# ssteinberg/wave_tracer

Measured on AMD Instinct MI355X. Metric: Msamples/sec (whole node), cornell-box 1440^2 wave-mode, higher is better.
Workload: dtype f32

## Files before the change

wave_tracer_amd/api.py:

```python
import ctypes as C
import json
import math
import os

_HERE = os.path.dirname(os.path.abspath(__file__))

os.environ.setdefault("HSA_KERNARG_POOL_SIZE", str(16 << 20))


def lib_path():
    return os.environ.get("WTGPU_LIB") or os.path.join(_HERE, "libwtgpu.so")


class WtgpuError(RuntimeError):
    pass


class SceneParams(C.Structure):
    _fields_ = [("res", C.c_uint32), ("max_depth", C.c_int32), ("fsd", C.c_int32), ("mis", C.c_int32), ("rr", C.c_int32),
                ("force_ray_tracing", C.c_int32), ("mesh_detail", C.c_int32), ("lut_n_theta", C.c_uint32), ("lut_m", C.c_uint32),
                ("polarimetric", C.c_int32)]


class TestHooks(C.Structure):
# ... 113 lines not shown
    lib.wtgpu_scene_compare_part.argtypes = [vp, vp, C.c_char_p, C.c_char_p, C.c_size_t]
    lib.wtgpu_trace_ab_stats.argtypes = [vp, C.POINTER(C.c_double), C.POINTER(C.c_double), C.POINTER(u64), C.POINTER(u64), C.POINTER(u64)]
    lib.wtgpu_render_progressive.argtypes = [vp, vp, vp, vp, vp, u64, u64, u64, u32, PROGRESS_CB, vp, C.POINTER(u64)]
    lib.wtgpu_cancel.argtypes = [vp]
    lib.wtgpu_pause.argtypes = [vp]
    lib.wtgpu_resume.argtypes = [vp]
    lib.wtgpu_capture_intermediate.argtypes = [vp, CAPTURE_CB, vp]
    lib.wtgpu_comm_unique_id.argtypes = [vp]
    lib.wtgpu_comm_create.argtypes = [i32, i32, i32, vp, C.POINTER(vp)]
    lib.wtgpu_film_reduce.argtypes = [vp, vp, vp, vp, vp, u64, u64, i32]
    lib.wtgpu_comm_destroy.argtypes = [vp]
    lib.wtgpu_comm_destroy.restype = None
    lib.wtgpu_scene_get_info.argtypes = [vp, C.POINTER(SceneInfo)]
    lib.wtgpu_scene_host_desc.argtypes = [vp]
    lib.wtgpu_scene_host_desc.restype = vp
    lib.wtgpu_scene_upload.argtypes = [vp, i32, u64]
    lib.wtgpu_render.argtypes = [vp, vp, vp, vp, vp, u64, u64, u64]
    lib.wtgpu_render_async.argtypes = [vp, vp, vp, vp, vp, u64, u64, u64]
    lib.wtgpu_join.argtypes = [vp, vp]
    lib.wtgpu_trace_rays.argtypes = [vp, vp, vp, u32, vp, vp, vp, vp]
    lib.wtgpu_traverse_cones.argtypes = [vp, vp, vp, u32, u32, vp, vp, vp, vp]
    lib.wtgpu_query_regions.argtypes = [vp, vp, vp, u32, u32, vp, vp, vp, vp, vp, vp, vp]
    lib.wtgpu_test_fsd_apertures.argtypes = [vp, vp, vp, vp, vp, vp, u32, u32, u32, u32, vp, vp]
    lib.wtgpu_test_utd_sums.argtypes = [vp, vp, vp, vp, vp, u32, u32, u32, vp, vp, vp]
    lib.wtgpu_test_profile_counters.argtypes = [vp, vp, u32]
    lib.wtgpu_test_bsdf_queries.argtypes = [vp, vp, vp, u32, i32, vp]
    lib.wtgpu_test_source_queries.argtypes = [vp, vp, vp, u32, vp]
    lib.wtgpu_scene_shape_id.argtypes = [vp, u32, C.POINTER(C.c_char_p)]
    lib.wtgpu_scene_sensor_mask_spec.argtypes = [vp, C.POINTER(SensorMaskSpec)]
    lib.wtgpu_sensor_mask.argtypes = [vp, vp, vp, u32, u64, vp]
    lib.wtgpu_sensor_mask_host.argtypes = [vp, vp, u32, u64, u32, vp]
    lib.wtgpu_scene_tonemap_spec.argtypes = [vp, C.POINTER(TonemapSpec)]
    lib.wtgpu_develop_device.argtypes = [vp, vp, vp, vp, vp, u64, vp]
    lib.wtgpu_tonemap_device.argtypes = [vp, vp, vp, vp, vp, u64, C.POINTER(Tonemap), u32, vp, u32, vp]
    lib.wtgpu_tonemap_host.argtypes = [vp, vp, vp, vp, u64, C.POINTER(Tonemap), u32, vp, u32, u32, vp]
    lib.wtgpu_film_stats_edges.argtypes = [C.POINTER(FilmStatsSpec), vp]
    lib.wtgpu_film_stats_device.argtypes = [vp, vp, vp, vp, vp, u64, C.POINTER(FilmStatsSpec), vp, vp, vp]
    lib.wtgpu_film_stats_host.argtypes = [vp, vp, vp, vp, u64, C.POINTER(FilmStatsSpec), vp, u32, vp, vp]
    lib.wtgpu_film_compare_device.argtypes = [vp, vp, vp, vp, vp, u64, vp, vp, vp, u64, C.POINTER(FilmCompareSpec), vp, vp, vp]
    lib.wtgpu_film_compare_host.argtypes = [vp, vp, vp, vp, u64, vp, vp, vp, u64, C.POINTER(FilmCompareSpec), vp, u32, vp, vp]
    lib.wtgpu_calibrate_copy.argtypes = [u64, i32]
    lib.wtgpu_get_counters.argtypes = [vp, C.POINTER(Counters)]
    lib.wtgpu_reset_counters.argtypes = [vp]
    lib.wtgpu_last_render_timings.argtypes = [vp, C.POINTER(C.c_float * 12)]
    lib.wtgpu_develop.argtypes = [vp, vp, vp, vp, u64, vp]
    lib.wtgpu_scene_destroy.argtypes = [vp]
# ... 173 lines not shown
        _check(load_library().wtgpu_traverse_cones(self._h, None, d_cones.data_ptr(), n, cap, dist.data_ptr(), flags.data_ptr(), ntris.data_ptr(),
                                                   tris.data_ptr()))
        torch.cuda.synchronize(dev)
        return (dist.cpu().numpy(), flags.cpu().numpy().view(np.uint32), ntris.cpu().numpy().view(np.uint32),
                tris.cpu().numpy().view(np.uint32))

    def query_regions(self, cones, edge_cap=96):
        import numpy as np
        import torch
        dev = torch.device("cuda", self.device)
        n = len(cones)
        d_cones = torch.from_numpy(np.ascontiguousarray(cones, dtype=np.float32)).to(dev)
        dist = torch.zeros(n, dtype=torch.float32, device=dev)
        flux = torch.zeros(n, dtype=torch.float32, device=dev)
        flags, primary, ntris, nedges = (torch.zeros(n, dtype=torch.int32, device=dev) for _ in range(4))
        edges = torch.full((n, edge_cap), -1, dtype=torch.int32, device=dev)
        _check(load_library().wtgpu_query_regions(self._h, None, d_cones.data_ptr(), n, edge_cap, dist.data_ptr(), flags.data_ptr(), primary.data_ptr(),
                                                  ntris.data_ptr(), nedges.data_ptr(), edges.data_ptr(), flux.data_ptr()))
        torch.cuda.synchronize(dev)
        u = lambda t: t.cpu().numpy().view(np.uint32)
        return {"dist": dist.cpu().numpy(), "flags": u(flags), "primary": u(primary), "ntris": u(ntris), "nedges": u(nedges), "edges": u(edges),
                "flux": flux.cpu().numpy()}

    def fsd_apertures(self, cones, sk, ids, n_ids, pool_cap=4096, mode=0):
        import numpy as np
        import torch
        dev = torch.device("cuda", self.device)
        ids = np.ascontiguousarray(ids, dtype=np.uint32)
        n, id_cap = ids.shape
        n_ids = np.ascontiguousarray(n_ids, dtype=np.uint32)
        assert len(cones) == n and len(sk) == n and len(n_ids) == n and (n_ids <= id_cap).all()
        n_edges = self.info.n_edges
        assert all((ids[i, :n_ids[i]] < n_edges).all() for i in range(n)), "edge id out of range"
        t = lambda a, dt: torch.from_numpy(np.ascontiguousarray(a, dtype=dt)).to(dev)
        d_cones, d_sk = t(cones, np.float32), t(sk, np.float32)
        d_ids, d_nids = t(ids.view(np.int32), np.int32), t(n_ids.view(np.int32), np.int32)
        hdr = torch.zeros((n, 8), dtype=torch.int32, device=dev)
        segs = torch.zeros((n, pool_cap, 7), dtype=torch.float32, device=dev)
        _check(load_library().wtgpu_test_fsd_apertures(self._h, None, d_cones.data_ptr(), d_sk.data_ptr(), d_ids.data_ptr(), d_nids.data_ptr(), n, id_cap,
                                                       pool_cap, mode, hdr.data_ptr(), segs.data_ptr()))
        torch.cuda.synchronize(dev)
        return hdr.cpu().numpy().view(np.uint32), segs.cpu().numpy()

    def utd_sums(self, queries, ids, n_ids, utd_cap=48):
        import numpy as np
        import torch
# ... 356 lines not shown
```

wave_tracer_amd/csrc/kernels_trace.hip:

```cpp
#include "wtgpu_kernels.h"

namespace wtk {

}
#include "kernels_trace_refill.h"
namespace wtk {

__global__ void __launch_bounds__(kBlock, WTGPU_LB_TRACE) k_trace_refill(launch_args_t a, int in, int first_round, uint32_t round) { trace_refill_body(a, in, first_round, round); }

#ifndef WTGPU_SM_EXACT_MIN
#define WTGPU_SM_EXACT_MIN 24
#endif
#ifndef WTGPU_SM_SPLIT_NODE
#define WTGPU_SM_SPLIT_NODE 0
#endif
#ifndef WTGPU_SM_BOTH
#define WTGPU_SM_BOTH 0
#endif
enum : int { PH_IDLE = 0, PH_NODE = 1, PH_TRI = 2, PH_EXACT = 3, PH_SERVE = 4, PH_POLICY = 5, PH_RAYDONE = 6 };
#ifdef WTGPU_SM_PROF
#define SP_DECL() unsigned long long sp_t[8] = {0, 0, 0, 0, 0, 0, 0, 0}, sp_l[8] = {0, 0, 0, 0, 0, 0, 0, 0}, sp_n[8] = {0, 0, 0, 0, 0, 0, 0, 0}; long long sp_c = 0
#define SP_BEGIN() sp_c = clock64()
#define SP_END(i, mask) do { const long long d_ = clock64() - sp_c; sp_t[i] += (unsigned long long)d_; sp_l[i] += (unsigned long long)d_ * (unsigned long long)__popcll(mask); sp_n[i] += 1; } while (0)
#else
// ... 769 lines not shown
        const range_t izr{tr.dist, tr.dist + tr.region_depth};
        prim = tr.tuid;
        const vec2 ax = cone_axes(env, tr.dist);
        ge = coop_gather(sc, env, izr, env, cone_frame(env), izr, vec2{1.f, 1.f}, false, gsh, false, true, nullptr, 1, &eg);
        __syncthreads();
        if (sc.n_edges <= kCoopEdgeBits) {
            ge.n_edges = coop_edge_count(sc, eg);
            coop_edge_write(sc, eg, edges + (size_t)i * edge_cap, edge_cap);
        } else
            for (uint32_t j = threadIdx.x; j < ge.n_edges && j < edge_cap; j += 64) edges[(size_t)i * edge_cap + j] = eg.edge_ids[j];
        __syncthreads();
        gf = coop_gather(sc, env, izr, env, cone_frame(env), izr, vec2{ax.x / kBeamEnvelope, ax.y / kBeamEnvelope}, tr.front_face != 0, gsh, true, false);
    }
    if (threadIdx.x == 0) {
        dist[i] = tr.dist;
        flags[i] = (tr.empty ? 1u : 0u) | (tr.ballistic ? 2u : 0u) | (tr.front_face ? 4u : 0u);
        primary[i] = prim;
        ntris[i] = gf.n_tris;
        nedges[i] = ge.n_edges + ge.edge_overflow;
        flux[i] = (float)gf.flux;
    }
}

}
```

wave_tracer_amd/csrc/wt/coop.h:

```cpp
#pragma once
#if defined(__HIPCC__)
#include "bvh.h"
#include "gauss.h"

namespace wt {

constexpr int kCoopStack = 512;
#ifndef WTGPU_COOP_LEAF_TRIS
#define WTGPU_COOP_LEAF_TRIS 256
#endif
constexpr uint32_t kCoopLeafTris = WTGPU_COOP_LEAF_TRIS;
constexpr uint32_t kCoopGatherLeafTris = 64;
constexpr uint32_t kCoopTriBuf = 64 + 8 * kCoopLeafTris;

#ifndef WTGPU_COOP_FLUSH_AT
#define WTGPU_COOP_FLUSH_AT 12
#endif
constexpr uint32_t kCoopFlushAt = WTGPU_COOP_FLUSH_AT;
constexpr uint32_t kCoopSurvCap = 128;

#ifndef WT_COOP_SPHERES
#define WT_COOP_SPHERES 1
#endif
#ifndef WT_COOP_SPHERE_PREFETCH
#define WT_COOP_SPHERE_PREFETCH 1
#endif
constexpr uint32_t kCoopSpherePrefetch = WT_COOP_SPHERE_PREFETCH;
WT_D const float4* coop_tri_spheres(const scene_t& sc) { return reinterpret_cast<const float4*>(sc.tri_geo + sc.n_tris); }
struct coop_shared_t {
    unsigned long long* dropped;
    stack_entry_t stack[kCoopStack];
    uint32_t tri_buf[kCoopTriBuf];
    uint32_t surv[kCoopSurvCap];
    float hit_dist[64];
};
struct coop_gather_shared_t {
    unsigned long long* dropped;
    stack_entry_t stack[kCoopStack];
    uint32_t tri_buf[64 + 8 * 64];
    uint32_t surv[kCoopSurvCap];
};
struct coop_edges_t {
    uint32_t edge_ids[96];
    uint32_t edge_bits[1024];
};
constexpr uint32_t kCoopEdgeBits = 32768;

template <class SH>
WT_D void coop_set_dropped_counter(SH& sh, unsigned long long* slot) {
    if (threadIdx.x == 0) sh.dropped = slot;
    __syncthreads();
}
WT_D float wave_min(float v) {
#pragma unroll
    for (int off = 32; off > 0; off >>= 1) v = fminf(v, __shfl_xor(v, off, 64));
    return v;
}
WT_D int uniform(int x) { return __builtin_amdgcn_readfirstlane(x); }
WT_D uint32_t uniform(uint32_t x) { return (uint32_t)__builtin_amdgcn_readfirstlane((int)x); }
WT_D bool uniform(bool x) { return __builtin_amdgcn_readfirstlane((int)x) != 0; }
WT_D float uniform(float x) { return __int_as_float(__builtin_amdgcn_readfirstlane(__float_as_int(x))); }
WT_D vec3 uniform(vec3 v) { return vec3{uniform(v.x), uniform(v.y), uniform(v.z)}; }
WT_D range_t uniform(const range_t& r) { return range_t{uniform(r.min), uniform(r.max)}; }
WT_D cone_t uniform(const cone_t& c) {
    cone_t u;
    u.o = uniform(c.o);
    u.d = uniform(c.d);
    u.x = uniform(c.x);
    u.x0 = uniform(c.x0);
    u.tan_alpha = uniform(c.tan_alpha);
    u.e = uniform(c.e);
    u.one_over_e = uniform(c.one_over_e);
    u.z_apex = uniform(c.z_apex);
    return u;
}

WT_D void coop_tri_vertices(const scene_t& sc, uint32_t tuid, vec3& a, vec3& b, vec3& c) {
    const float4* q = reinterpret_cast<const float4*>(sc.tri_geo + tuid);
    const float4 q0 = q[0], q1 = q[1];
    const float q2 = reinterpret_cast<const float*>(q)[8];
    a = vec3{q0.x, q0.y, q0.z};
    b = vec3{q0.w, q1.x, q1.y};
    c = vec3{q1.z, q1.w, q2};
}

WT_D bool cone_child_test(const bvh8_node_t& n, int i, vec3 ro, vec3 rd, vec3 rinvd, bool sx, bool sy, bool sz, float ta, float ix,
                                       const range_t& range, float& tmin_out) {
    float ominx = n.minx[i] - ro.x, ominy = n.miny[i] - ro.y, ominz = n.minz[i] - ro.z;
    float omaxx = n.maxx[i] - ro.x, omaxy = n.maxy[i] - ro.y, omaxz = n.maxz[i] - ro.z;
    const bool outside = cone_box_outside(ominx, ominy, ominz, omaxx, omaxy, omaxz, rd, ta, ix, range);
    const float bx = sx ? ominx : omaxx, by = sy ? ominy : omaxy, bz = sz ? ominz : omaxz;
    const float dot_d_b = rd.x * bx + rd.y * by + rd.z * bz;
    const float maxz = clampf(dot_d_b, 0.f, range.max);
    const float enlr = fmaf(maxz, ta, ix);
    ominx -= enlr;
    ominy -= enlr;
    ominz -= enlr;
    omaxx += enlr;
    omaxy += enlr;
    omaxz += enlr;
    const float dminx = (sx ? omaxx : ominx) * rinvd.x, dmaxx = (sx ? ominx : omaxx) * rinvd.x;
    const float dminy = (sy ? omaxy : ominy) * rinvd.y, dmaxy = (sy ? ominy : omaxy) * rinvd.y;
    const float dminz = (sz ? omaxz : ominz) * rinvd.z, dmaxz = (sz ? ominz : omaxz) * rinvd.z;
    float tmin = 0.f, tmax = dmaxx;
    tmin = fmaxf_(tmin, dminx);
    tmax = fminf_(tmax, dmaxy);
    tmin = fmaxf_(tmin, dminy);
    tmax = fminf_(tmax, dmaxz);
    tmin = fmaxf_(tmin, dminz);
    tmin_out = tmin;
    return !outside && tmin <= tmax && tmax >= range.min && tmin <= range.max && !(tmin >= range.max);
}

template <bool any_hit>
WT_D bool coop_cone_query(const scene_t& sc, const cone_t& cone_, const range_t& searchrange_, float z_scale, coop_shared_t& sh,
                                       const uint_list_t& tris, cone_hit_t& rec, unsigned long long* prof = nullptr, float min_progress_ = -WT_INF) {
    const cone_t cone = uniform(cone_);
    const range_t searchrange = uniform(searchrange_);
    const float min_progress = uniform(min_progress_);
    const int lane = threadIdx.x & 63;
    const int grp = lane >> 3, sub = lane & 7;
    rec.dist = WT_INF;
    rec.front_face = 0;
    rec.ntris = 0;
    rec.overflow = 0;
    rec.aborted = 0;
    rec.too_short = 0;
    rec.short_tuid = kInvalid;
    if (sc.n_nodes == 0) return false;
    const vec3 ro = cone.o, rd = cone.d;
    const vec3 rinvd = uniform(vec3{1.f / rd.x, 1.f / rd.y, 1.f / rd.z});
    const bool sx = __builtin_signbit(rinvd.x), sy = __builtin_signbit(rinvd.y), sz = __builtin_signbit(rinvd.z);
    const float ta = cone.tan_alpha, ix = cone.x0;
    range_t range = any_hit ? searchrange : uniform(cone_search_range(cone, searchrange, rec.dist, z_scale));
    float slab_max = range.max;
    int s = 1;
    uint32_t leaf_total = 0, nsurv = 0;
    if (lane == 0) sh.stack[0] = stack_entry_t{0.f, 1};
    __syncthreads();
    auto compact = [&](float zmax) __attribute__((always_inline)) {
        if (rec.ntris == 0) return;
        __syncthreads();
        const bool mine = (uint32_t)lane < rec.ntris;
        const uint32_t val = mine ? tris[lane] : 0u;
        const float dv = mine ? sh.hit_dist[lane] : 0.f;
        const bool keep = mine && !(dv > zmax);
        const unsigned long long km = __ballot(keep);
        __syncthreads();
        if (keep) {
            const uint32_t np_ = (uint32_t)__popcll(km & ((1ull << lane) - 1ull));
            tris[np_] = val;
            sh.hit_dist[np_] = dv;
        }
        rec.ntris = (uint32_t)__popcll(km);
        __syncthreads();
    };
    auto flush = [&]() __attribute__((always_inline)) -> bool {
        __syncthreads();
        bool any = false;
        for (uint32_t b2 = 0; b2 < nsurv && !any; b2 += 64) {
// ... 105 lines not shown
            CP(1);
            const unsigned long long hm = __ballot(h);
            if (hm) {
                const uint32_t gbits = (uint32_t)(hm >> (grp * 8)) & 0xffu;
                int rank = 0;
#pragma unroll
                for (int j = 0; j < 8; ++j) {
                    const float tj = __shfl(tmin, (lane & ~7) + j, 64);
                    if (((gbits >> j) & 1u) && (tj > tmin || (tj == tmin && j < sub))) ++rank;
                }
                const int above = grp < 7 ? __popcll(hm >> ((grp + 1) * 8)) : 0;
                const int pos = s + above + rank;
                if (h && pos < kCoopStack) sh.stack[pos] = stack_entry_t{tmin, cp};
                else if (h) atomicAdd(sh.dropped, 1ull);
                const int total = s + __popcll(hm);
                s = total < kCoopStack ? total : kCoopStack;
            }
            CP(2);
            const unsigned long long lm = __ballot(leafish && sub == 0 && cnt > 0);
            unsigned long long m = lm;
            while (m) {
                const int src = __ffsll((long long)m) - 1;
                m &= m - 1;
                uint32_t c = uniform((uint32_t)__shfl((int)cnt, src, 64));
                const uint32_t t = uniform((uint32_t)__shfl((int)t0, src, 64));
                if (c > kCoopLeafTris) c = kCoopLeafTris;
                for (uint32_t q = (uint32_t)lane; q < c; q += 64u) sh.tri_buf[leaf_total + q] = t + q;
                leaf_total += c;
            }
            __syncthreads();
            CP(3);
        }
        if (prof) prof[5] += (unsigned long long)(clock64() - ta0);
        const long long tb0 = prof ? clock64() : 0;
        bool found_any = false;
#ifdef WTGPU_COOP_PROF
        if (prof) { prof[10] += 1; prof[11] += leaf_total; prof[8] += (leaf_total + 63u) / 64u; }
#endif
#if WT_COOP_SPHERES
        {
            const float4* spheres = coop_tri_spheres(sc);
            uint32_t n2 = 0;
            for (uint32_t base0 = 0; base0 < leaf_total; base0 += 64u * kCoopSpherePrefetch) {
                float4 bs[kCoopSpherePrefetch];
                uint32_t tu[kCoopSpherePrefetch];
#pragma unroll
                for (uint32_t j = 0; j < kCoopSpherePrefetch; ++j) {
                    const uint32_t k = base0 + 64u * j + lane;
                    tu[j] = 0;
                    bs[j] = float4{0.f, 0.f, 0.f, 0.f};
                    if (k < leaf_total) {
                        tu[j] = sh.tri_buf[k];
                        bs[j] = spheres[tu[j]];
                    }
                }
#pragma unroll
                for (uint32_t j = 0; j < kCoopSpherePrefetch; ++j) asm volatile("" : "+v"(bs[j].x), "+v"(bs[j].y), "+v"(bs[j].z), "+v"(bs[j].w));
                __syncthreads();
#pragma unroll
                for (uint32_t j = 0; j < kCoopSpherePrefetch; ++j) {
                    const uint32_t k = base0 + 64u * j + lane;
// ... 8 lines not shown
            CP(7);
        }
#endif
        for (uint32_t base = 0; base < leaf_total && !found_any; base += 64) {
            const uint32_t k = base + lane;
            bool pass = false;
            uint32_t tuid = 0;
            if (k < leaf_total) {
                tuid = sh.tri_buf[k];
                vec3 va, vb, vc;
                coop_tri_vertices(sc, tuid, va, vb, vc);
                pass = cone_tri_maybe(cone, va, vb, vc, range);
            }
            const unsigned long long pm = __ballot(pass);
            if (pm) {
                const uint32_t pos = nsurv + (uint32_t)__popcll(pm & ((1ull << lane) - 1ull));
                if (pass && pos < kCoopSurvCap) sh.surv[pos] = tuid;
                nsurv += (uint32_t)__popcll(pm);
            }
            CP(7);
            if (nsurv >= 64u) found_any = flush();
            CP(6);
        }
        leaf_total = 0;
        CP(7);
        if (!found_any && nsurv > 0 && (s == 0 || nsurv >= kCoopFlushAt)) found_any = flush();
        CP(6);
        __syncthreads();
        if (prof) prof[6] += (unsigned long long)(clock64() - tb0);
        if (found_any && (any_hit || rec.too_short)) return true;
        if (s == 0) break;
    }
    return rec.ntris > 0;
}

WT_D void coop_cone(const scene_t& sc, const cone_t& cone, const range_t& searchrange, float z_scale, coop_shared_t& sh,
                                 const uint_list_t& tris, cone_hit_t& rec, unsigned long long* prof = nullptr, float min_progress = -WT_INF) {
    coop_cone_query<false>(sc, cone, searchrange, z_scale, sh, tris, rec, prof, min_progress);
}
WT_D bool coop_cone_any(const scene_t& sc, const cone_t& cone, const range_t& range, coop_shared_t& sh, unsigned long long* prof = nullptr,
                                     uint32_t* hit_tuid = nullptr) {
    cone_hit_t rec;
    const uint_list_t none{nullptr, 0, 0};
    const bool hit = coop_cone_query<true>(sc, cone, range, 0.f, sh, none, rec, prof);
    if (hit_tuid) *hit_tuid = rec.short_tuid;
    return hit;
}

struct gather_out_t {
    double flux;
    uint32_t n_edges, edge_overflow;
    uint32_t n_tris;
};
template <class SH>
WT_D gather_out_t coop_gather(const scene_t& sc, const cone_t& tcone, const range_t& slab, const cone_t& envelope, const frame_t& beam_frame,
                                           const range_t& izr, vec2 sigma, bool want_front, SH& sh, bool do_flux, bool do_edges,
                                           unsigned long long* stats = nullptr, int32_t root = 1, coop_edges_t* eg = nullptr) {
    uint32_t* edges = eg ? eg->edge_ids : nullptr;
    const uint32_t edge_cap = 96;
    const int lane = threadIdx.x & 63;
    const int grp = lane >> 3, sub = lane & 7;
    gather_out_t out{0.0, 0u, 0u, 0u};
    const bool edges_only = do_edges && !do_flux;
// ... 229 lines not shown
        float tmin = 0.f;
        if (grp < np) {
            const bvh8_node_t& node = sc.nodes[e.ptr - 1];
            cp = node.child[sub];
            if (cp != 0 && cone_child_test(node, sub, ro, rd, rinvd, sx, sy, sz, ta, ix, slab, tmin)) {
                if (cp < 0 || sc.nodes[cp - 1].tris_count <= max_tris)
                    emit(cp);
                else
                    push = true;
            }
        }
        const unsigned long long hm = __ballot(push);
        if (hm) {
            const int pos = s + __popcll(hm & ((1ull << lane) - 1ull));
            if (push && pos < kCoopStack) sh.stack[pos] = stack_entry_t{tmin, cp};
            else if (push) emit(cp);
            const int total = s + __popcll(hm);
            s = total < kCoopStack ? total : kCoopStack;
        }
        __syncthreads();
    }
}

WT_D bool coop_ray_query(const scene_t& sc, vec3 ro_, vec3 rd_, const range_t& range_, coop_shared_t& sh, ray_hit_t& rec) {
    const vec3 ro = uniform(ro_), rd = uniform(rd_);
    const range_t range = uniform(range_);
    const int lane = threadIdx.x & 63;
    const int grp = lane >> 3, sub = lane & 7;
    rec.dist = WT_INF;
    rec.tuid = kInvalid;
    rec.bx = rec.by = 0.f;
    rec.front_face = 0;
    if (sc.n_nodes == 0) return false;
    const vec3 rinvd = uniform(vec3{1.f / rd.x, 1.f / rd.y, 1.f / rd.z});
    const bool sx = __builtin_signbit(rinvd.x), sy = __builtin_signbit(rinvd.y), sz = __builtin_signbit(rinvd.z);
    int s = 1;
    uint32_t leaf_total = 0;
    if (lane == 0) sh.stack[0] = stack_entry_t{0.f, 1};
    __syncthreads();
    for (;;) {
        while (s > 0 && leaf_total < 64u) {
            const int np = s < 8 ? s : 8;
            stack_entry_t e{0.f, 0};
            if (grp < np) e = sh.stack[s - 1 - grp];
            s -= np;
            __syncthreads();
            const bool live = grp < np && e.t < rec.dist;
            bool leafish = false, h = false;
            uint32_t t0 = 0, cnt = 0;
            float tmin = 0.f;
            int32_t cp = 0;
            if (live) {
                if (e.ptr < 0) {
                    const bvh8_leaf_t leaf = bvh_leaf_of(e.ptr);
                    t0 = leaf.tris_ptr;
                    cnt = leaf.count;
                    leafish = true;
                } else {
                    const bvh8_node_t& n = sc.nodes[e.ptr - 1];
                    const uint32_t ntc = n.tris_count, nts = n.tris_start;
// ... 21 lines not shown
                }
            }
            const unsigned long long hm = __ballot(h);
            if (hm) {
                const uint32_t gbits = (uint32_t)(hm >> (grp * 8)) & 0xffu;
                int rank = 0;
#pragma unroll
                for (int j = 0; j < 8; ++j) {
                    const float tj = __shfl(tmin, (lane & ~7) + j, 64);
                    if (((gbits >> j) & 1u) && (tj > tmin || (tj == tmin && j < sub))) ++rank;
                }
                const int above = grp < 7 ? __popcll(hm >> ((grp + 1) * 8)) : 0;
                const int pos = s + above + rank;
                if (h && pos < kCoopStack) sh.stack[pos] = stack_entry_t{tmin, cp};
                else if (h) atomicAdd(sh.dropped, 1ull);
                const int total = s + __popcll(hm);
                s = total < kCoopStack ? total : kCoopStack;
            }
            const unsigned long long lm = __ballot(leafish && sub == 0 && cnt > 0);
            unsigned long long m = lm;
            while (m) {
                const int src = __ffsll((long long)m) - 1;
                m &= m - 1;
                uint32_t c = uniform((uint32_t)__shfl((int)cnt, src, 64));
                const uint32_t t = uniform((uint32_t)__shfl((int)t0, src, 64));
                if (c > kCoopLeafTris) c = kCoopLeafTris;
                for (uint32_t q = (uint32_t)lane; q < c; q += 64u) sh.tri_buf[leaf_total + q] = t + q;
                leaf_total += c;
            }
            __syncthreads();
        }
        if (leaf_total == 0) {
            if (s == 0) break;
            continue;
        }
        for (uint32_t base = 0; base < leaf_total; base += 64) {
            const uint32_t k = base + lane;
            bool hit = false;
            float d = WT_INF;
            uint32_t tuid = 0;
            ray_tri_hit_t ht{WT_INF, 0.f, 0.f};
            bool ff = false;
            if (k < leaf_total) {
                tuid = sh.tri_buf[k];
                const tri_geo_t tri = sc.tri_geo[tuid];
                if (intersect_ray_tri_wide(ro, rd, tri.a, tri.b, tri.c, range, ht) && ht.dist < rec.dist) {
                    hit = true;
                    d = ht.dist;
                    ff = dot(tri.n, rd) <= 0.f;
                }
            }
            const unsigned long long mask = __ballot(hit);
            if (mask) {
                const float dm = uniform(wave_min(d));
                const unsigned long long m2 = __ballot(hit && d == dm);
                const int src = __ffsll((long long)m2) - 1;
                rec.dist = dm;
                rec.tuid = uniform((uint32_t)__shfl((int)tuid, src, 64));
                rec.bx = uniform(__shfl(ht.bx, src, 64));
                rec.by = uniform(__shfl(ht.by, src, 64));
                rec.front_face = uniform((uint32_t)__shfl((int)ff, src, 64));
            }
        }
        leaf_total = 0;
        __syncthreads();
        if (s == 0) break;
    }
    if (!finitef(rec.dist) || rec.dist > range.max) {
        rec.dist = WT_INF;
        return false;
    }
    return true;
}

WT_D trav_result_t coop_traverse(const scene_t& sc, const cone_t& envelope_, float lambda_m_, float distance_, bool force_ray_tracing,
                                              coop_shared_t& sh, const uint_list_t& tris, unsigned long long* prof = nullptr, bool resume = false,
                                              uint32_t seg0_ = 0, float dist0 = 0.f, uint32_t nray0 = 0, uint32_t ncone0 = 0, const ray_hit_t* axis = nullptr,
                                              bool primary_always = false, bool probe_resumed = true, uint32_t short_tuid_ = kInvalid,
                                              uint32_t origin_tuid_ = kInvalid, bool use_cache = true) {
    const cone_t envelope = uniform(envelope_);
    const float lambda_m = uniform(lambda_m_), distance = uniform(distance_);
    const uint32_t seg0 = uniform(seg0_), origin_tuid = uniform(origin_tuid_);
    uint32_t short_tuid = uniform(short_tuid_);
#ifdef WTGPU_COOP_PROF
#define WT_COOP_PROF(i, t0_)
#else
#define WT_COOP_PROF(i, t0_) \
    if (prof) prof[i] += (unsigned long long)(clock64() - (t0_));
#endif
    trav_result_t r;
    r.aborted = 0;
    r.origin = envelope.o;
    r.empty = 1;
    r.ballistic = 1;
    r.dist = -WT_INF;
    r.region_depth = 0.f;
    r.front_face = 0;
    r.tuid = kInvalid;
    r.bx = r.by = 0.f;
// ... 91 lines not shown
```

wave_tracer_amd/csrc/wtgpu_kernels.h:

```cpp
#pragma once
#include <hip/hip_runtime.h>

#include <cstddef>
#include <cstdint>
#include <cstring>

#include "../../include/wtgpu.h"
#include "wt/bdpt.h"
#include "wt/coop.h"
#include "wt/coop_fsd.h"
#include "wt/coop_utd.h"
#include "wt/path.h"

using namespace wt;
namespace wt {
struct tonemap_args_t;
}

namespace wtk {


#ifndef WTGPU_LB_TRACE
#define WTGPU_LB_TRACE 3
#endif
// ... 297 lines not shown
__global__ void k_path_fsd(launch_args_t a, const path_state_t* __restrict__ ps, uint32_t round);
__global__ void k_path_edges(launch_args_t a, const path_state_t* __restrict__ ps);
__global__ void k_path_interact(launch_args_t a, const path_state_t* __restrict__ ps, int in, int first_round, uint32_t round);
__global__ void k_path_interact_b(launch_args_t a, const path_state_t* __restrict__ ps, int in, uint32_t round);
__global__ void k_path_nee(launch_args_t a, const path_state_t* __restrict__ ps, uint32_t round);
__global__ void k_path_flush(launch_args_t a, int in);
__global__ void k_connect_enum(launch_args_t a, uint32_t by_class);
__global__ void k_connect_scan(launch_args_t a, uint32_t by_class);
__global__ void k_connect_strat(launch_args_t a);
__global__ void k_connect_strat_open(launch_args_t a);
__global__ void k_connect_class(launch_args_t a);
__global__ void k_connect_class_open(launch_args_t a);
__global__ void k_connect_eval(launch_args_t a, uint32_t chunk);
__global__ void k_connect_shadow(launch_args_t a, uint32_t chunk);
__global__ void k_connect_mis(launch_args_t a, uint32_t chunk);
__global__ void k_connect_splat(launch_args_t a);
__global__ void k_connect_splat_tiled(launch_args_t a);
__global__ void k_calib_copy(const uint32_t* in, uint32_t* out, size_t n);
__global__ void k_trace_rays(scene_t sc, const float* rays, uint32_t n, float* dist, uint32_t* tuid, float* bary, uint32_t* front);
__global__ void k_traverse_cones(scene_t sc, const float* cones, uint32_t n, uint32_t cap, float* dist, uint32_t* flags, uint32_t* ntris, uint32_t* out_tris,
                                 uint32_t* scratch_tris);
__global__ void k_query_regions(scene_t sc, const float* cones, uint32_t n, uint32_t edge_cap, float* dist, uint32_t* flags, uint32_t* primary, uint32_t* ntris,
                                uint32_t* nedges, uint32_t* edges, float* flux, unsigned long long* dropped);
int test_fsd_apertures(const scene_t& sc, hipStream_t stream, const float* d_cones, const float* d_sk, const uint32_t* d_ids, const uint32_t* d_n_ids,
                       uint32_t n, uint32_t id_cap, uint32_t pool_cap, uint32_t mode, uint32_t* d_hdr, float* d_segs);
int test_utd_sums(const scene_t& sc, hipStream_t stream, const float* d_queries, const uint32_t* d_ids, const uint32_t* d_n_ids, uint32_t n, uint32_t id_cap,
                  uint32_t utd_cap, uint32_t* d_recs, uint32_t* d_hdr, uint32_t* d_edges);
int test_bsdf_queries(const scene_t& sc, hipStream_t stream, const uint32_t* d_queries, uint32_t n, int form, uint32_t* d_out);
int test_source_queries(const scene_t& sc, hipStream_t stream, const uint32_t* d_queries, uint32_t n, uint32_t* d_out);
int sensor_mask_launch(const scene_t& sc, hipStream_t stream, const uint8_t* d_shape_matches, uint32_t samples, uint64_t seed, float* d_out);
void sensor_mask_host(const scene_t& sc, const uint8_t* shape_matches, uint32_t samples, uint64_t seed, uint32_t n_threads, float* out);
constexpr uint32_t kMaxTonemapTable = 1024;
int develop_launch(const sensor_t& sn, hipStream_t stream, const double* d_value, const double* d_weight, const double* d_light, uint64_t spe,
                   uint32_t per_pixel, float* d_out);
int develop_tonemap_launch(const sensor_t& sn, hipStream_t stream, const double* d_value, const double* d_weight, const double* d_light, uint64_t spe,
                           const tonemap_args_t& t, uint32_t s, const float* d_mask, uint32_t format, uint32_t lds_table, void* d_out);
void develop_tonemap_host(const sensor_t& sn, const double* value, const double* weight, const double* light, uint64_t spe, const tonemap_args_t& t, uint32_t s,
                          const float* mask, uint32_t format, uint32_t n_threads, void* out);
int film_stats_launch(const sensor_t& sn, hipStream_t stream, uint32_t n_cus, const double* d_value, const double* d_weight, const double* d_light, uint64_t spe, uint32_t s,
                      uint32_t flags, const float* d_mask, const float* d_edges, uint32_t bins, void* d_rec, unsigned long long* d_hist, double* d_sums);
void film_stats_host(const sensor_t& sn, const double* value, const double* weight, const double* light, uint64_t spe, uint32_t s, uint32_t flags, const float* mask,
                     const float* edges, uint32_t bins, uint32_t n_threads, void* out_rec, unsigned long long* out_hist);
size_t film_compare_wave_bytes(uint64_t npix, uint32_t n_cus);
int film_compare_launch(const sensor_t& sn, hipStream_t stream, uint32_t n_cus, const double* a_value, const double* a_weight, const double* a_light, uint64_t spe_a,
                        const double* b_value, const double* b_weight, const double* b_light, uint64_t spe_b, uint32_t s, uint32_t flags, double eps, const float* d_mask,
                        void* d_rec, double* d_sums, void* d_wave, float* d_diff);
// ... 7 lines not shown
```

wave_tracer_amd/csrc/wtgpu_queries.hip:

```cpp
#include "wtgpu_host.h"
#include "wt/sources_probe.h"

extern "C" {

int wtgpu_trace_rays(wtgpu_scene* s, void* stream_, const float* d_rays, uint32_t n, float* d_dist, uint32_t* d_tuid, float* d_bary, uint32_t* d_front) {
    if (!s || !s->uploaded) return fail(WTGPU_ERR_INVALID, "scene not uploaded");
    hipStream_t stream = static_cast<hipStream_t>(stream_);
    hipLaunchKernelGGL(k_trace_rays, dim3((n + kBlock - 1) / kBlock), dim3(kBlock), 0, stream, s->dev, d_rays, n, d_dist, d_tuid, d_bary, d_front);
    HIP_CHECK(hipGetLastError());
    return WTGPU_OK;
}
int wtgpu_traverse_cones(wtgpu_scene* s, void* stream_, const float* d_cones, uint32_t n, uint32_t cap, float* d_dist, uint32_t* d_flags,
                         uint32_t* d_ntris, uint32_t* d_tris) {
    if (!s || !s->uploaded) return fail(WTGPU_ERR_INVALID, "scene not uploaded");
    hipStream_t stream = static_cast<hipStream_t>(stream_);
    const size_t need = (size_t)n * kMaxConeTris * 4 * 2;
    if (need > s->query_scratch_bytes) {
        device_guard_t guard(s->device);
        void* p = nullptr;
        HIP_CHECK(hipMalloc(&p, need));
        s->dev_allocs.push_back(p);
        s->query_scratch = static_cast<uint32_t*>(p);
        s->query_scratch_bytes = need;
    }
    hipLaunchKernelGGL(k_traverse_cones, dim3((n + kBlock - 1) / kBlock), dim3(kBlock), 0, stream, s->dev, d_cones, n, cap, d_dist, d_flags, d_ntris,
                       d_tris, s->query_scratch);
    HIP_CHECK(hipGetLastError());
    return WTGPU_OK;
}

int wtgpu_query_regions(wtgpu_scene* s, void* stream_, const float* d_cones, uint32_t n, uint32_t edge_cap, float* d_dist, uint32_t* d_flags,
                        uint32_t* d_primary, uint32_t* d_ntris, uint32_t* d_nedges, uint32_t* d_edges, float* d_flux) {
    if (!s || !s->uploaded) return fail(WTGPU_ERR_INVALID, "scene not uploaded");
    if (n == 0) return WTGPU_OK;
    hipLaunchKernelGGL(k_query_regions, dim3(n), dim3(64), 0, static_cast<hipStream_t>(stream_), s->dev, d_cones, n, edge_cap, d_dist, d_flags, d_primary,
                       d_ntris, d_nedges, d_edges, d_flux, s->slices[0].counters + kDroppedSlot);
    HIP_CHECK(hipGetLastError());
    return WTGPU_OK;
}

int wtgpu_scene_shape_id(const wtgpu_scene* s, uint32_t shape, const char** id) {
    if (!s || !id) return fail(WTGPU_ERR_INVALID, "null argument");
    if (shape >= s->host.n_shapes) return fail(WTGPU_ERR_INVALID, "shape index out of range");
    *id = shape < s->file.shape_ids.size() ? s->file.shape_ids[shape].c_str() : "";
    return WTGPU_OK;
}
int wtgpu_scene_sensor_mask_spec(const wtgpu_scene* s, wtgpu_sensor_mask_spec* out) {
    if (!s || !out) return fail(WTGPU_ERR_INVALID, "null argument");
    out->present = s->file.has_mask ? 1 : 0;
    out->samples = s->file.mask_samples;
    out->regex = s->file.mask_regex.c_str();
    out->shape_flags = s->file.has_mask && !s->file.mask_flags.empty() ? s->file.mask_flags.data() : nullptr;
    out->n_shapes = s->host.n_shapes;
    return WTGPU_OK;
}
static int mask_flags_for(const wtgpu_scene* s, const uint8_t* shape_flags, uint32_t samples, const uint8_t** flags) {
    if (s->host.sensor.type != SENSOR_PERSPECTIVE)
        return fail(WTGPU_ERR_INVALID, "sensor masks need a perspective sensor (only the perspective loader reads a <sensor_mask>: src/sensor/perspective.cpp:98)");
    if (samples == 0 || samples > 65536) return fail(WTGPU_ERR_INVALID, "sensor mask: 1 .. 65536 samples per pixel expected");
// ... 126 lines not shown
```

wave_tracer_amd/csrc/wtgpu_test_hooks.h:

```cpp
#pragma once
#include "../../include/wtgpu.h"
#ifdef __cplusplus
extern "C" {
#endif
typedef struct wtgpu_test_hooks {
    uint32_t only_s, only_t;
    uint32_t crop_of;
} wtgpu_test_hooks;
int wtgpu_scene_create_named_hooks(const char* name, const wtgpu_scene_params* params, const wtgpu_test_hooks* hooks, wtgpu_scene** out);
int wtgpu_scene_compare(const wtgpu_scene* a, const wtgpu_scene* b, char* what, size_t n_what);
int wtgpu_scene_compare_part(const wtgpu_scene* a, const wtgpu_scene* b, const char* part, char* what, size_t n_what);
int wtgpu_trace_ab_stats(wtgpu_scene* s, double* ms_refill, double* ms_sm, uint64_t* differing_words, uint64_t* walks, uint64_t* rounds);
int wtgpu_test_profile_counters(wtgpu_scene* s, unsigned long long* out, uint32_t n);
int wtgpu_test_fsd_apertures(wtgpu_scene* s, void* stream, const float* d_cones, const float* d_sk, const uint32_t* d_ids, const uint32_t* d_n_ids,
                             uint32_t n, uint32_t id_cap, uint32_t pool_cap, uint32_t mode, uint32_t* d_hdr, float* d_segs);
int wtgpu_test_utd_sums(wtgpu_scene* s, void* stream, const float* d_queries, const uint32_t* d_ids, const uint32_t* d_n_ids, uint32_t n, uint32_t id_cap,
                        uint32_t utd_cap, uint32_t* d_recs, uint32_t* d_hdr, uint32_t* d_edges);
int wtgpu_test_bsdf_queries(wtgpu_scene* s, void* stream, const uint32_t* d_queries, uint32_t n, int form, uint32_t* d_out);
int wtgpu_test_source_queries(wtgpu_scene* s, void* stream, const uint32_t* d_queries, uint32_t n, uint32_t* d_out);
int wtgpu_test_connect_class_order(uint32_t* keys, uint32_t cap, uint32_t* n_keys, uint32_t* key_dim);
int wtgpu_test_connect_class_items(wtgpu_scene* s, uint32_t slice, uint32_t* table, uint32_t* items, uint32_t items_cap, uint32_t* n_items);
#ifdef __cplusplus
}
#endif
```

Before: 32.65.

## Replace explicit per-leaf triangle id buffer with wave-register leaf ranges in coop traversal

```diff
diff --git a/wave_tracer_amd/api.py b/wave_tracer_amd/api.py
--- a/wave_tracer_amd/api.py
+++ b/wave_tracer_amd/api.py
@@ -159,6 +159,8 @@
     lib.wtgpu_traverse_cones.argtypes = [vp, vp, vp, u32, u32, vp, vp, vp, vp]
     lib.wtgpu_query_regions.argtypes = [vp, vp, vp, u32, u32, vp, vp, vp, vp, vp, vp, vp]
     lib.wtgpu_test_fsd_apertures.argtypes = [vp, vp, vp, vp, vp, vp, u32, u32, u32, u32, vp, vp]
+    if hasattr(lib, "wtgpu_test_heavy_queries"):
+        lib.wtgpu_test_heavy_queries.argtypes = [vp, vp, vp, u32, i32, vp, vp]
     lib.wtgpu_test_utd_sums.argtypes = [vp, vp, vp, vp, vp, u32, u32, u32, vp, vp, vp]
     lib.wtgpu_test_profile_counters.argtypes = [vp, vp, u32]
     lib.wtgpu_test_bsdf_queries.argtypes = [vp, vp, vp, u32, i32, vp]
@@ -378,6 +380,20 @@
         return {"dist": dist.cpu().numpy(), "flags": u(flags), "primary": u(primary), "ntris": u(ntris), "nedges": u(nedges), "edges": u(edges),
                 "flux": flux.cpu().numpy()}
 
+    def heavy_queries(self, queries, parent_form=False):
+        import numpy as np
+        import torch
+        dev = torch.device("cuda", self.device)
+        q = np.ascontiguousarray(queries, dtype=np.float32)
+        assert q.ndim == 2 and q.shape[1] == 16
+        n = len(q)
+        d_q = torch.from_numpy(q).to(dev)
+        out = torch.zeros((n, 8), dtype=torch.int32, device=dev)
+        tris = torch.zeros((n, 64), dtype=torch.int32, device=dev)
+        _check(load_library().wtgpu_test_heavy_queries(self._h, None, d_q.data_ptr(), n, int(bool(parent_form)), out.data_ptr(), tris.data_ptr()))
+        torch.cuda.synchronize(dev)
+        return out.cpu().numpy().view(np.uint32), tris.cpu().numpy().view(np.uint32)
+
     def fsd_apertures(self, cones, sk, ids, n_ids, pool_cap=4096, mode=0):
         import numpy as np
         import torch
diff --git a/wave_tracer_amd/csrc/kernels_trace.hip b/wave_tracer_amd/csrc/kernels_trace.hip
--- a/wave_tracer_amd/csrc/kernels_trace.hip
+++ b/wave_tracer_amd/csrc/kernels_trace.hip
@@ -815,4 +815,51 @@
     }
 }
 
-}
+template <class SH>
+WT_D void test_heavy_query(const scene_t& sc, const float* q, uint32_t i, uint32_t* out, uint32_t* tris, SH& sh) {
+    const float* c = q + 16 * (size_t)i;
+    const vec3 d = normalize(vec3{c[3], c[4], c[5]});
+    const cone_t env = uniform(make_cone(vec3{c[0], c[1], c[2]}, d, build_orthogonal_frame(d).t, c[6], c[8], c[7]));
+    const uint_list_t list{tris + (size_t)i * kMaxConeTris, 1u, kMaxConeTris};
+    for (uint32_t j = threadIdx.x; j < kMaxConeTris; j += 64) list[j] = kInvalid;
+    __syncthreads();
+    uint32_t o[8] = {0, 0, 0, 0, 0, kInvalid, 0, 0};
+    if (c[10] == 0.f) {
+        const trav_result_t tr = coop_traverse(sc, env, uniform(c[9]), WT_INF, false, sh, list);
+        o[0] = __float_as_uint(tr.dist);
+        o[1] = (tr.empty ? 1u : 0u) | (tr.ballistic ? 2u : 0u) | (tr.front_face ? 4u : 0u);
+        o[2] = tr.ballistic ? 0u : tr.ntris;
+        o[3] = tr.overflow;
+        o[6] = tr.n_cone_queries;
+        o[7] = tr.n_ray_queries;
+    } else {
+        cone_hit_t rec;
+        coop_cone_query<false>(sc, env, range_t{uniform(c[11]), uniform(c[12])}, kMajorAxisToZScale, sh, list, rec, nullptr, uniform(c[13]));
+        o[0] = __float_as_uint(rec.dist);
+        o[1] = rec.front_face ? 4u : 0u;
+        o[2] = rec.ntris;
+        o[3] = rec.overflow;
+        o[4] = rec.too_short;
+        o[5] = rec.short_tuid;
+        o[6] = 1;
+    }
+    __syncthreads();
+    for (uint32_t j = threadIdx.x; j < kMaxConeTris; j += 64)
+        if (j >= o[2]) list[j] = kInvalid;
+    if (threadIdx.x == 0)
+        for (int j = 0; j < 8; ++j) out[8 * (size_t)i + j] = o[j];
+}
+__global__ void __launch_bounds__(64) k_test_heavy_queries(scene_t sc, const float* q, uint32_t n, uint32_t* out, uint32_t* tris, unsigned long long* dropped) {
+    __shared__ coop_shared_t sh;
+    coop_set_dropped_counter(sh, dropped);
+    if (blockIdx.x < n) test_heavy_query(sc, q, blockIdx.x, out, tris, sh);
+}
+#if WTGPU_COOP_PARENT_FORM
+__global__ void __launch_bounds__(64) k_test_heavy_queries_ids(scene_t sc, const float* q, uint32_t n, uint32_t* out, uint32_t* tris, unsigned long long* dropped) {
+    __shared__ coop_shared_ids_t sh;
+    coop_set_dropped_counter(sh, dropped);
+    if (blockIdx.x < n) test_heavy_query(sc, q, blockIdx.x, out, tris, sh);
+}
+#endif
+
+}
diff --git a/wave_tracer_amd/csrc/wt/coop.h b/wave_tracer_amd/csrc/wt/coop.h
--- a/wave_tracer_amd/csrc/wt/coop.h
+++ b/wave_tracer_amd/csrc/wt/coop.h
@@ -27,13 +27,28 @@
 #endif
 constexpr uint32_t kCoopSpherePrefetch = WT_COOP_SPHERE_PREFETCH;
 WT_D const float4* coop_tri_spheres(const scene_t& sc) { return reinterpret_cast<const float4*>(sc.tri_geo + sc.n_tris); }
+constexpr uint32_t kCoopCandCap = 128;
 struct coop_shared_t {
+    static constexpr bool kExplicitIds = false;
+    unsigned long long* dropped;
+    stack_entry_t stack[kCoopStack];
+    uint32_t cand[kCoopCandCap];
+    uint32_t surv[kCoopSurvCap];
+    float hit_dist[64];
+};
+#ifndef WTGPU_COOP_PARENT_FORM
+#define WTGPU_COOP_PARENT_FORM 1
+#endif
+#if WTGPU_COOP_PARENT_FORM
+struct coop_shared_ids_t {
+    static constexpr bool kExplicitIds = true;
     unsigned long long* dropped;
     stack_entry_t stack[kCoopStack];
     uint32_t tri_buf[kCoopTriBuf];
     uint32_t surv[kCoopSurvCap];
     float hit_dist[64];
 };
+#endif
 struct coop_gather_shared_t {
     unsigned long long* dropped;
     stack_entry_t stack[kCoopStack];
@@ -74,6 +89,43 @@
     u.z_apex = uniform(c.z_apex);
     return u;
 }
+
+struct coop_ranges_t {
+    uint32_t t0 = 0, s0 = 0, t1 = 0, s1 = 0;
+    uint32_t n = 0;
+    uint32_t cur = 0;
+    WT_D void clear() { n = cur = 0; }
+    WT_D void push(uint32_t first, uint32_t start, int lane) {
+        const bool mine = (uint32_t)lane == (n & 63u);
+        if (n < 64u) {
+            t0 = mine ? first : t0;
+            s0 = mine ? start : s0;
+        } else {
+            t1 = mine ? first : t1;
+            s1 = mine ? start : s1;
+        }
+        ++n;
+    }
+    WT_D uint32_t first(uint32_t r) const {
+        return (uint32_t)(r < 64u ? __builtin_amdgcn_readlane((int)t0, (int)r) : __builtin_amdgcn_readlane((int)t1, (int)(r - 64u) & 63));
+    }
+    WT_D uint32_t start(uint32_t r, uint32_t total) const {
+        if (r >= n) return total;
+        return (uint32_t)(r < 64u ? __builtin_amdgcn_readlane((int)s0, (int)r) : __builtin_amdgcn_readlane((int)s1, (int)(r - 64u) & 63));
+    }
+    WT_D uint32_t fetch(uint32_t base, uint32_t total, int lane) {
+        const uint32_t k = base + (uint32_t)lane, bend = base + 64u < total ? base + 64u : total;
+        uint32_t tu = 0;
+        while (cur < n) {
+            const uint32_t S = start(cur, total), E = start(cur + 1u, total), T = first(cur);
+            if (k >= S && k < E) tu = T + (k - S);
+            if (E > bend) break;
+            ++cur;
+            if (E == bend) break;
+        }
+        return tu;
+    }
+};
 
 WT_D void coop_tri_vertices(const scene_t& sc, uint32_t tuid, vec3& a, vec3& b, vec3& c) {
     const float4* q = reinterpret_cast<const float4*>(sc.tri_geo + tuid);
@@ -112,8 +164,8 @@
     return !outside && tmin <= tmax && tmax >= range.min && tmin <= range.max && !(tmin >= range.max);
 }
 
-template <bool any_hit>
-WT_D bool coop_cone_query(const scene_t& sc, const cone_t& cone_, const range_t& searchrange_, float z_scale, coop_shared_t& sh,
+template <bool any_hit, class SH>
+WT_D bool coop_cone_query(const scene_t& sc, const cone_t& cone_, const range_t& searchrange_, float z_scale, SH& sh,
                                        const uint_list_t& tris, cone_hit_t& rec, unsigned long long* prof = nullptr, float min_progress_ = -WT_INF) {
     const cone_t cone = uniform(cone_);
     const range_t searchrange = uniform(searchrange_);
@@ -136,6 +188,7 @@
     float slab_max = range.max;
     int s = 1;
     uint32_t leaf_total = 0, nsurv = 0;
+    coop_ranges_t rg;
     if (lane == 0) sh.stack[0] = stack_entry_t{0.f, 1};
     __syncthreads();
     auto compact = [&](float zmax) __attribute__((always_inline)) {
@@ -287,11 +340,18 @@
             while (m) {
                 const int src = __ffsll((long long)m) - 1;
                 m &= m - 1;
-                uint32_t c = uniform((uint32_t)__shfl((int)cnt, src, 64));
-                const uint32_t t = uniform((uint32_t)__shfl((int)t0, src, 64));
-                if (c > kCoopLeafTris) c = kCoopLeafTris;
-                for (uint32_t q = (uint32_t)lane; q < c; q += 64u) sh.tri_buf[leaf_total + q] = t + q;
-                leaf_total += c;
+                if constexpr (SH::kExplicitIds) {
+                    uint32_t c = uniform((uint32_t)__shfl((int)cnt, src, 64));
+                    const uint32_t t = uniform((uint32_t)__shfl((int)t0, src, 64));
+                    if (c > kCoopLeafTris) c = kCoopLeafTris;
+                    for (uint32_t q = (uint32_t)lane; q < c; q += 64u) sh.tri_buf[leaf_total + q] = t + q;
+                    leaf_total += c;
+                } else {
+                    uint32_t c = (uint32_t)__builtin_amdgcn_readlane((int)cnt, src);
+                    if (c > kCoopLeafTris) c = kCoopLeafTris;
+                    rg.push((uint32_t)__builtin_amdgcn_readlane((int)t0, src), leaf_total, lane);
+                    leaf_total += c;
+                }
             }
             __syncthreads();
             CP(3);
@@ -302,6 +362,57 @@
 #ifdef WTGPU_COOP_PROF
         if (prof) { prof[10] += 1; prof[11] += leaf_total; prof[8] += (leaf_total + 63u) / 64u; }
 #endif
+        if constexpr (!SH::kExplicitIds) {
+            const float4* spheres = coop_tri_spheres(sc);
+            const range_t range_a = range;
+            uint32_t ncand = 0, chead = 0;
+            auto filter_batch = [&](uint32_t nb) __attribute__((always_inline)) {
+                __syncthreads();
+                bool pass = false;
+                uint32_t tuid = 0;
+                if ((uint32_t)lane < nb) {
+                    tuid = sh.cand[(chead + (uint32_t)lane) & (kCoopCandCap - 1u)];
+                    vec3 va, vb, vc;
+                    coop_tri_vertices(sc, tuid, va, vb, vc);
+                    pass = cone_tri_maybe(cone, va, vb, vc, range);
+                }
+                __syncthreads();
+                const unsigned long long pm = __ballot(pass);
+                if (pm) {
+                    const uint32_t pos = nsurv + (uint32_t)__popcll(pm & ((1ull << lane) - 1ull));
+                    if (pass && pos < kCoopSurvCap) sh.surv[pos] = tuid;
+                    nsurv += (uint32_t)__popcll(pm);
+                }
+                CP(7);
+                if (nsurv >= 64u) found_any = flush();
+                CP(6);
+            };
+            for (uint32_t base0 = 0; !found_any; base0 += 64u) {
+                const bool more = base0 < leaf_total;
+                if (more) {
+                    const uint32_t tu = rg.fetch(base0, leaf_total, lane);
+                    bool p1 = base0 + (uint32_t)lane < leaf_total;
+#if WT_COOP_SPHERES
+                    float4 bs{0.f, 0.f, 0.f, 0.f};
+                    if (p1) bs = spheres[tu];
+                    asm volatile("" : "+v"(bs.x), "+v"(bs.y), "+v"(bs.z), "+v"(bs.w));
+                    p1 = p1 && cone_sphere_maybe(cone, vec3{bs.x, bs.y, bs.z}, bs.w, range_a);
+#endif
+                    const unsigned long long pm1 = __ballot(p1);
+                    if (p1) sh.cand[(chead + ncand + (uint32_t)__popcll(pm1 & ((1ull << lane) - 1ull))) & (kCoopCandCap - 1u)] = tu;
+                    ncand += (uint32_t)__popcll(pm1);
+                    CP(7);
+                }
+                if (ncand >= 64u || (!more && ncand > 0)) {
+                    const uint32_t nb = ncand < 64u ? ncand : 64u;
+                    filter_batch(nb);
+                    chead = (chead + nb) & (kCoopCandCap - 1u);
+                    ncand -= nb;
+                }
+                if (!more) break;
+            }
+            rg.clear();
+        } else {
 #if WT_COOP_SPHERES
         {
             const float4* spheres = coop_tri_spheres(sc);
@@ -356,6 +467,7 @@
             if (nsurv >= 64u) found_any = flush();
             CP(6);
         }
+        }
         leaf_total = 0;
         CP(7);
         if (!found_any && nsurv > 0 && (s == 0 || nsurv >= kCoopFlushAt)) found_any = flush();
@@ -368,11 +480,13 @@
     return rec.ntris > 0;
 }
 
-WT_D void coop_cone(const scene_t& sc, const cone_t& cone, const range_t& searchrange, float z_scale, coop_shared_t& sh,
+template <class SH>
+WT_D void coop_cone(const scene_t& sc, const cone_t& cone, const range_t& searchrange, float z_scale, SH& sh,
                                  const uint_list_t& tris, cone_hit_t& rec, unsigned long long* prof = nullptr, float min_progress = -WT_INF) {
     coop_cone_query<false>(sc, cone, searchrange, z_scale, sh, tris, rec, prof, min_progress);
 }
-WT_D bool coop_cone_any(const scene_t& sc, const cone_t& cone, const range_t& range, coop_shared_t& sh, unsigned long long* prof = nullptr,
+template <class SH>
+WT_D bool coop_cone_any(const scene_t& sc, const cone_t& cone, const range_t& range, SH& sh, unsigned long long* prof = nullptr,
                                      uint32_t* hit_tuid = nullptr) {
     cone_hit_t rec;
     const uint_list_t none{nullptr, 0, 0};
@@ -648,7 +762,8 @@
     }
 }
 
-WT_D bool coop_ray_query(const scene_t& sc, vec3 ro_, vec3 rd_, const range_t& range_, coop_shared_t& sh, ray_hit_t& rec) {
+template <class SH>
+WT_D bool coop_ray_query(const scene_t& sc, vec3 ro_, vec3 rd_, const range_t& range_, SH& sh, ray_hit_t& rec) {
     const vec3 ro = uniform(ro_), rd = uniform(rd_);
     const range_t range = uniform(range_);
     const int lane = threadIdx.x & 63;
@@ -662,6 +777,7 @@
     const bool sx = __builtin_signbit(rinvd.x), sy = __builtin_signbit(rinvd.y), sz = __builtin_signbit(rinvd.z);
     int s = 1;
     uint32_t leaf_total = 0;
+    coop_ranges_t rg;
     if (lane == 0) sh.stack[0] = stack_entry_t{0.f, 1};
     __syncthreads();
     for (;;) {
@@ -729,11 +845,18 @@
             while (m) {
                 const int src = __ffsll((long long)m) - 1;
                 m &= m - 1;
-                uint32_t c = uniform((uint32_t)__shfl((int)cnt, src, 64));
-                const uint32_t t = uniform((uint32_t)__shfl((int)t0, src, 64));
-                if (c > kCoopLeafTris) c = kCoopLeafTris;
-                for (uint32_t q = (uint32_t)lane; q < c; q += 64u) sh.tri_buf[leaf_total + q] = t + q;
-                leaf_total += c;
+                if constexpr (SH::kExplicitIds) {
+                    uint32_t c = uniform((uint32_t)__shfl((int)cnt, src, 64));
+                    const uint32_t t = uniform((uint32_t)__shfl((int)t0, src, 64));
+                    if (c > kCoopLeafTris) c = kCoopLeafTris;
+                    for (uint32_t q = (uint32_t)lane; q < c; q += 64u) sh.tri_buf[leaf_total + q] = t + q;
+                    leaf_total += c;
+                } else {
+                    uint32_t c = (uint32_t)__builtin_amdgcn_readlane((int)cnt, src);
+                    if (c > kCoopLeafTris) c = kCoopLeafTris;
+                    rg.push((uint32_t)__builtin_amdgcn_readlane((int)t0, src), leaf_total, lane);
+                    leaf_total += c;
+                }
             }
             __syncthreads();
         }
@@ -748,8 +871,9 @@
             uint32_t tuid = 0;
             ray_tri_hit_t ht{WT_INF, 0.f, 0.f};
             bool ff = false;
+            if constexpr (!SH::kExplicitIds) tuid = rg.fetch(base, leaf_total, lane);
             if (k < leaf_total) {
-                tuid = sh.tri_buf[k];
+                if constexpr (SH::kExplicitIds) tuid = sh.tri_buf[k];
                 const tri_geo_t tri = sc.tri_geo[tuid];
                 if (intersect_ray_tri_wide(ro, rd, tri.a, tri.b, tri.c, range, ht) && ht.dist < rec.dist) {
                     hit = true;
@@ -770,6 +894,7 @@
             }
         }
         leaf_total = 0;
+        rg.clear();
         __syncthreads();
         if (s == 0) break;
     }
@@ -780,8 +905,9 @@
     return true;
 }
 
+template <class SH>
 WT_D trav_result_t coop_traverse(const scene_t& sc, const cone_t& envelope_, float lambda_m_, float distance_, bool force_ray_tracing,
-                                              coop_shared_t& sh, const uint_list_t& tris, unsigned long long* prof = nullptr, bool resume = false,
+                                              SH& sh, const uint_list_t& tris, unsigned long long* prof = nullptr, bool resume = false,
                                               uint32_t seg0_ = 0, float dist0 = 0.f, uint32_t nray0 = 0, uint32_t ncone0 = 0, const ray_hit_t* axis = nullptr,
                                               bool primary_always = false, bool probe_resumed = true, uint32_t short_tuid_ = kInvalid,
                                               uint32_t origin_tuid_ = kInvalid, bool use_cache = true) {
diff --git a/wave_tracer_amd/csrc/wtgpu_kernels.h b/wave_tracer_amd/csrc/wtgpu_kernels.h
--- a/wave_tracer_amd/csrc/wtgpu_kernels.h
+++ b/wave_tracer_amd/csrc/wtgpu_kernels.h
@@ -343,6 +343,10 @@
                                  uint32_t* scratch_tris);
 __global__ void k_query_regions(scene_t sc, const float* cones, uint32_t n, uint32_t edge_cap, float* dist, uint32_t* flags, uint32_t* primary, uint32_t* ntris,
                                 uint32_t* nedges, uint32_t* edges, float* flux, unsigned long long* dropped);
+__global__ void k_test_heavy_queries(scene_t sc, const float* q, uint32_t n, uint32_t* out, uint32_t* tris, unsigned long long* dropped);
+#if WTGPU_COOP_PARENT_FORM
+__global__ void k_test_heavy_queries_ids(scene_t sc, const float* q, uint32_t n, uint32_t* out, uint32_t* tris, unsigned long long* dropped);
+#endif
 int test_fsd_apertures(const scene_t& sc, hipStream_t stream, const float* d_cones, const float* d_sk, const uint32_t* d_ids, const uint32_t* d_n_ids,
                        uint32_t n, uint32_t id_cap, uint32_t pool_cap, uint32_t mode, uint32_t* d_hdr, float* d_segs);
 int test_utd_sums(const scene_t& sc, hipStream_t stream, const float* d_queries, const uint32_t* d_ids, const uint32_t* d_n_ids, uint32_t n, uint32_t id_cap,
diff --git a/wave_tracer_amd/csrc/wtgpu_queries.hip b/wave_tracer_amd/csrc/wtgpu_queries.hip
--- a/wave_tracer_amd/csrc/wtgpu_queries.hip
+++ b/wave_tracer_amd/csrc/wtgpu_queries.hip
@@ -35,6 +35,23 @@
     if (n == 0) return WTGPU_OK;
     hipLaunchKernelGGL(k_query_regions, dim3(n), dim3(64), 0, static_cast<hipStream_t>(stream_), s->dev, d_cones, n, edge_cap, d_dist, d_flags, d_primary,
                        d_ntris, d_nedges, d_edges, d_flux, s->slices[0].counters + kDroppedSlot);
+    HIP_CHECK(hipGetLastError());
+    return WTGPU_OK;
+}
+
+int wtgpu_test_heavy_queries(wtgpu_scene* s, void* stream_, const float* d_queries, uint32_t n, int parent_form, uint32_t* d_out, uint32_t* d_tris) {
+    if (!s || !s->uploaded) return fail(WTGPU_ERR_INVALID, "scene not uploaded");
+    if (n == 0) return WTGPU_OK;
+    if (!d_queries || !d_out || !d_tris) return fail(WTGPU_ERR_INVALID, "null argument");
+    unsigned long long* dropped = s->slices[0].counters + kDroppedSlot;
+    if (parent_form) {
+#if WTGPU_COOP_PARENT_FORM
+        hipLaunchKernelGGL(k_test_heavy_queries_ids, dim3(n), dim3(64), 0, static_cast<hipStream_t>(stream_), s->dev, d_queries, n, d_out, d_tris, dropped);
+#else
+        return fail(WTGPU_ERR_INVALID, "wtgpu_test_heavy_queries: built with WTGPU_COOP_PARENT_FORM=0, the explicit-id form is not in this library");
+#endif
+    } else
+        hipLaunchKernelGGL(k_test_heavy_queries, dim3(n), dim3(64), 0, static_cast<hipStream_t>(stream_), s->dev, d_queries, n, d_out, d_tris, dropped);
     HIP_CHECK(hipGetLastError());
     return WTGPU_OK;
 }
diff --git a/wave_tracer_amd/csrc/wtgpu_test_hooks.h b/wave_tracer_amd/csrc/wtgpu_test_hooks.h
--- a/wave_tracer_amd/csrc/wtgpu_test_hooks.h
+++ b/wave_tracer_amd/csrc/wtgpu_test_hooks.h
@@ -18,6 +18,7 @@
                         uint32_t utd_cap, uint32_t* d_recs, uint32_t* d_hdr, uint32_t* d_edges);
 int wtgpu_test_bsdf_queries(wtgpu_scene* s, void* stream, const uint32_t* d_queries, uint32_t n, int form, uint32_t* d_out);
 int wtgpu_test_source_queries(wtgpu_scene* s, void* stream, const uint32_t* d_queries, uint32_t n, uint32_t* d_out);
+int wtgpu_test_heavy_queries(wtgpu_scene* s, void* stream, const float* d_queries, uint32_t n, int parent_form, uint32_t* d_out, uint32_t* d_tris);
 int wtgpu_test_connect_class_order(uint32_t* keys, uint32_t cap, uint32_t* n_keys, uint32_t* key_dim);
 int wtgpu_test_connect_class_items(wtgpu_scene* s, uint32_t slice, uint32_t* table, uint32_t* items, uint32_t items_cap, uint32_t* n_items);
 #ifdef __cplusplus
```

Result: no change. 32.38 (median of 2 runs) (-0.8%).
